# vliu15/3d-brain-tumor-segmentation

Hardware: AMD Instinct MI355X
Metric: training volumes/sec (2ch x 128^3) (higher is better)
Workload: dtype f32; 1 GPU; BASELINE configs[1]: 2ch x 128^3, batch 1 per GPU, fp32, full fwd+bwd with Dice+KL+L2 VAE loss + Dice metric + TF-form Adam; CLI-default model (base_filters=32, depth=4, groups=8, reduction=8; 42,174,773 params); parallelism=dp1, global_batch=1

## Files before the change

### 3d-brain-tumor-segmentation_amd/csrc/conv_c2.hip

```cpp
#include <stdlib.h>
#include "common.h"
#include "conv_plan.h"

struct C2Params {
  const float* x;
  const float* wp;
  const float* bias;
  float* y;
  const float* wp2;
  const float* bias2;
  float* y2;
  int N, D, H, W, ldx, Cout, ldy, ldy2, Npad;
  int ntz, nty, ntx;
  double* gnp;
  int gn_G, gn_zt;
};

template <bool F2>
__global__ __launch_bounds__(256, 2) void c2_kernel(const C2Params p) {
  __shared__ float lds[2 * 6 * 6 * 34 + 16];
  const int tid = threadIdx.x;
  const int lane = tid & 63;
  const int wave = __builtin_amdgcn_readfirstlane(tid >> 6);
  const int h = lane >> 5, l32 = lane & 31;
  int b = blockIdx.x;
  const int tx = b % p.ntx; b /= p.ntx;
  const int ty = b % p.nty; b /= p.nty;
  const int tz = b % p.ntz;
  const int n = b / p.ntz;
  const int oz0 = tz * 4, oy0 = ty * 4, ox0 = tx * 32;
  for (int e = tid; e < 6 * 6 * 34; e += 256) {
    const int vz = e / (6 * 34), r = e - vz * (6 * 34);
    const int vy = r / 34, vx = r - vy * 34;
    const int z = oz0 - 1 + vz, yy = oy0 - 1 + vy, xx = ox0 - 1 + vx;
    float v0 = 0.f, v1 = 0.f;
    if ((unsigned)z < (unsigned)p.D && (unsigned)yy < (unsigned)p.H && (unsigned)xx < (unsigned)p.W) {
      const float* s = p.x + ((((long)n * p.D + z) * p.H + yy) * p.W + xx) * (long)p.ldx;
      v0 = s[0]; v1 = s[1];
    }
    lds[e] = v0;
    lds[6 * 6 * 34 + e] = v1;
  }
  float wt[27];
#pragma unroll
  for (int t = 0; t < 27; ++t) wt[t] = p.wp[((long)t * 2 * p.Npad + l32) * 4 + h];
  float w2 = 0.f;
  if (F2) w2 = p.wp2[l32 * 4 + h];
  __syncthreads();
  f32x16 acc[4], acc2[F2 ? 4 : 1];
#pragma unroll
  for (int i = 0; i < 4; ++i)
#pragma unroll
    for (int r = 0; r < 16; ++r) { acc[i][r] = 0.f; if (F2) acc2[F2 ? i : 0][r] = 0.f; }
  const float* lb = lds + h * (6 * 6 * 34) + (wave * 6) * 34 + l32;
#pragma unroll
  for (int kz = 0; kz < 3; ++kz) {
    float f[6][3];
#pragma unroll
    for (int yr = 0; yr < 6; ++yr)
#pragma unroll
      for (int kx = 0; kx < 3; ++kx) f[yr][kx] = lb[(kz * 6 + yr) * 34 + kx];
#pragma unroll
    for (int ky = 0; ky < 3; ++ky)
#pragma unroll
      for (int kx = 0; kx < 3; ++kx)
#pragma unroll
        for (int oy = 0; oy < 4; ++oy)
          acc[oy] = __builtin_amdgcn_mfma_f32_32x32x2f32(wt[(kz * 3 + ky) * 3 + kx], f[oy + ky][kx], acc[oy], 0, 0, 0);
    if (F2 && kz == 1) {
#pragma unroll
      for (int oy = 0; oy < 4; ++oy) acc2[F2 ? oy : 0] = __builtin_amdgcn_mfma_f32_32x32x2f32(w2, f[oy + 1][1], acc2[F2 ? oy : 0], 0, 0, 0);
    }
  }
  const int oz = oz0 + wave, ox = ox0 + l32;
  float gn_s = 0.f, gn_q = 0.f;
  if (oz < p.D && ox < p.W) {
#pragma unroll
    for (int oy = 0; oy < 4; ++oy) {
      const int y = oy0 + oy;
      if (y >= p.H) continue;
      const long pix = (((long)n * p.D + oz) * p.H + y) * p.W + ox;
#pragma unroll
      for (int g = 0; g < 4; ++g) {
        const int co = 8 * g + 4 * h;
        if (co >= p.Cout) continue;
        f32x4 v = {acc[oy][4 * g], acc[oy][4 * g + 1], acc[oy][4 * g + 2], acc[oy][4 * g + 3]};
        if (p.bias) {
#pragma unroll
          for (int j = 0; j < 4; ++j) v[j] += p.bias[co + j];
        }
        if (p.gnp) {
#pragma unroll
          for (int j = 0; j < 4; ++j) { gn_s += v[j]; gn_q = fmaf(v[j], v[j], gn_q); }
        }
        *reinterpret_cast<f32x4*>(p.y + pix * p.ldy + co) = v;
        if (F2) {
          f32x4 v2 = {acc2[F2 ? oy : 0][4 * g], acc2[F2 ? oy : 0][4 * g + 1], acc2[F2 ? oy : 0][4 * g + 2], acc2[F2 ? oy : 0][4 * g + 3]};
          if (p.bias2) {
#pragma unroll
            for (int j = 0; j < 4; ++j) v2[j] += p.bias2[co + j];
          }
          *reinterpret_cast<f32x4*>(p.y2 + pix * p.ldy2 + co) = v2;
        }
      }
    }
  }
  if (p.gnp) {
    const double ds = wave_sum_f64((double)gn_s), dq = wave_sum_f64((double)gn_q);
    __syncthreads();
    double* sh = reinterpret_cast<double*>(lds);
    if (lane == 0) { sh[wave * 2] = ds; sh[wave * 2 + 1] = dq; }
    __syncthreads();
    if (tid == 0) {
      const int g = tz / p.gn_zt;
      const long B = (long)p.gn_zt * p.nty * p.ntx;
      const long b_ = ((long)(tz - g * p.gn_zt) * p.nty + ty) * p.ntx + tx;
      double* o = p.gnp + (((long)n * p.gn_G + g) * B + b_) * 2;
      o[0] = sh[0] + sh[2] + sh[4] + sh[6];
      o[1] = sh[1] + sh[3] + sh[5] + sh[7];
    }
  }
}

static inline long c2_tiles(const ConvCall& c, int& ntx, int& nty, int& ntz) {
  ntx = (c.Wi + 31) / 32; nty = (c.Hi + 3) / 4; ntz = (c.Di + 3) / 4;
  return (long)c.N * ntz * nty * ntx;
}
bool c2_accept(const ConvCall& c, ConvChoice& ch) {
  if (c.Cin != 2 || c.Cout > 32 || c.Cout % 4 != 0 || c.ldy % 4 != 0 || !c.y16) return false;
  if (c.flags & (IG_FLAG_ACCUM | IG_FLAG_SIGMOID)) return false;
  if (c.second == CONV_Y2 && (c.ld2 % 4 != 0 || !c.p2_16)) return false;
  int ntx, nty, ntz;
  const long tiles = c2_tiles(c, ntx, nty, ntz);
  if (tiles < conv_env_long("BTS_IGEMM_C2_MIN", 512) || tiles > 0x7fffffffL) return false;
  ch.sym = SYM_C2;
  ch.gn_B = (long)conv_gn_zt(c, 4) * nty * ntx;
  return true;
}
int bts_c2_launch_(const ConvCall& c, const ConvChoice& ch, const ConvPtrs& q, hipStream_t stream) {
  const bool f2 = c.second == CONV_Y2;
  C2Params p;
  p.x = q.x; p.wp = q.wp; p.bias = (c.flags & IG_FLAG_BIAS) ? q.bias : nullptr; p.y = q.y;
  p.wp2 = f2 ? q.wp2 : nullptr; p.bias2 = f2 ? q.bias2 : nullptr; p.y2 = f2 ? q.y2 : nullptr;
  p.N = c.N; p.D = c.Di; p.H = c.Hi; p.W = c.Wi; p.ldx = c.ldx; p.Cout = c.Cout; p.ldy = c.ldy; p.ldy2 = f2 ? c.ld2 : 0; p.Npad = conv_npad32(c.Cout);
  const long tiles = c2_tiles(c, p.ntx, p.nty, p.ntz);
  p.gnp = ch.gn_B ? q.gnp : nullptr; p.gn_G = ch.gn_B ? c.G : 0; p.gn_zt = ch.gn_B ? (c.Di / c.G) / 4 : 1;
  const bool prof = bts_prof_on();
  if (prof) bts_prof_begin(ch.sym, 2.0 * (27.0 + (f2 ? 1.0 : 0.0)) * c.Cin * (double)c.Cout * (double)c.N * c.Di * c.Hi * c.Wi, stream);
  (void)hipGetLastError();
  if (f2) hipLaunchKernelGGL(c2_kernel<true>, dim3((unsigned)tiles), dim3(256), 0, stream, p);
  else hipLaunchKernelGGL(c2_kernel<false>, dim3((unsigned)tiles), dim3(256), 0, stream, p);
  if (prof) bts_prof_end(stream);
  BTS_LAUNCH_CHECK();
  return BTS_OK;
}
```

### 3d-brain-tumor-segmentation_amd/csrc/conv_dsc.hip

```cpp
#include <stdlib.h>
#include "common.h"
#include "conv_plan.h"

struct DscParams {
  const float* x;
  const float* wp;
  const float* bias;
  float* y;
  int N, D, H, W, Cin, ldx, Cout, ldy, Npad, KG, ntx, nty, ntz, flags;
};
template <int CO>
__global__ __launch_bounds__(256, 4) void dsc_kernel(const DscParams p) {
  constexpr int S = 12, TX = 32, TY = 4, TZ = 2, IX = TX + 2, IY = TY + 2, IZ = TZ + 2;
  constexpr int tileVox = IZ * IY * IX, nslots = tileVox * 2, NSL = (nslots + 255) / 256;
  __shared__ __attribute__((aligned(16))) float lds[tileVox * S];
  const int tid = threadIdx.x;
  int b = blockIdx.x;
  const int tx = b % p.ntx; b /= p.ntx;
  const int ty = b % p.nty; b /= p.nty;
  const int tz = b % p.ntz;
  const int n = b / p.ntz;
  const int iz0 = tz * TZ - 1, iy0 = ty * TY - 1, ix0 = tx * TX - 1;
  const float* xbase = p.x + ((((long)n * p.D + iz0) * p.H + iy0) * p.W + ix0) * (long)p.ldx;
  int goff[NSL];
#pragma unroll
  for (int i = 0; i < NSL; ++i) {
    const int e = tid + i * 256;
    goff[i] = -1;
    if (e < nslots) {
      const int vox = e >> 1, q = e & 1;
      const int vz = vox / (IY * IX), r = vox - vz * (IY * IX), vy = r / IX, vx = r - vy * IX;
      if ((unsigned)(iz0 + vz) < (unsigned)p.D && (unsigned)(iy0 + vy) < (unsigned)p.H && (unsigned)(ix0 + vx) < (unsigned)p.W)
        goff[i] = ((vz * p.H + vy) * p.W + vx) * p.ldx + q * 4;
    }
  }
  const int mx = tid & (TX - 1), my = (tid >> 5) & (TY - 1), mz = tid >> 7;
  const float* lb = lds + ((mz * IY + my) * IX + mx) * S;
  float acc[CO];
#pragma unroll
  for (int c = 0; c < CO; ++c) acc[c] = 0.f;
  const int wstepKG = 2 * p.Npad * 4, wstepTap = p.KG * wstepKG;
  f32x4 pre[NSL];
  auto fetch = [&](int kg) {
#pragma unroll
    for (int i = 0; i < NSL; ++i) {
      f32x4 v = {0.f, 0.f, 0.f, 0.f};
      if (goff[i] >= 0) v = *reinterpret_cast<const f32x4*>(xbase + goff[i] + kg * 8);
      pre[i] = v;
    }
  };
  fetch(0);
  for (int kg = 0; kg < p.KG; ++kg) {
    __syncthreads();
#pragma unroll
    for (int i = 0; i < NSL; ++i) {
      const int e = tid + i * 256;
      if (e < nslots) *reinterpret_cast<f32x4*>(lds + (e >> 1) * S + (e & 1) * 4) = pre[i];
    }
    __syncthreads();
    if (kg + 1 < p.KG) fetch(kg + 1);
    const float* wk = p.wp + kg * wstepKG;
#pragma unroll
    for (int r = 0; r < 9; ++r) {
      float w[3][2][CO * 4];
#pragma unroll
      for (int dx = 0; dx < 3; ++dx)
#pragma unroll
        for (int hh = 0; hh < 2; ++hh)
#pragma unroll
          for (int q = 0; q < CO * 4; ++q) w[dx][hh][q] = wk[(r * 3 + dx) * wstepTap + hh * p.Npad * 4 + q];
      f32x4 xv[3][2];
#pragma unroll
      for (int dx = 0; dx < 3; ++dx) {
        const float* src = lb + (((r / 3) * IY + r % 3) * IX + dx) * S;
        xv[dx][0] = *reinterpret_cast<const f32x4*>(src);
        xv[dx][1] = *reinterpret_cast<const f32x4*>(src + 4);
      }
      __builtin_amdgcn_sched_barrier(0);
#pragma unroll
      for (int dx = 0; dx < 3; ++dx)
#pragma unroll
        for (int hh = 0; hh < 2; ++hh)
#pragma unroll
          for (int c = 0; c < CO; ++c)
#pragma unroll
            for (int j = 0; j < 4; ++j) acc[c] = fmaf(xv[dx][hh][j], w[dx][hh][c * 4 + j], acc[c]);
      __builtin_amdgcn_sched_barrier(0);
    }
  }
  const int oz = tz * TZ + mz, oy = ty * TY + my, ox = tx * TX + mx;
  if (oz >= p.D || oy >= p.H || ox >= p.W) return;
  float* yrow = p.y + ((((long)n * p.D + oz) * p.H + oy) * p.W + ox) * (long)p.ldy;
#pragma unroll
  for (int c = 0; c < CO; ++c) {
    if (c < p.Cout) {
      float v = acc[c];
      if (p.flags & IG_FLAG_BIAS) v += p.bias[c];
      if (p.flags & IG_FLAG_SIGMOID) v = sigmoidf_(v);
      if (p.flags & IG_FLAG_ACCUM) v += yrow[c];
      yrow[c] = v;
    }
  }
}

static inline long dsc_tiles(const ConvCall& c, int& ntx, int& nty, int& ntz) {
  ntx = (c.Wi + 31) / 32; nty = (c.Hi + 3) / 4; ntz = (c.Di + 1) / 2;
  return (long)c.N * ntz * nty * ntx;
}
bool dsc_accept(const ConvCall& c, ConvChoice& ch) {
  if (c.Cout > 4 || (c.Cin & 7) || (c.ldx & 3) || !c.x16) return false;
  int ntx, nty, ntz;
  const long tiles = dsc_tiles(c, ntx, nty, ntz);
  ch.sym = SYM_DSC;
  return tiles >= conv_env_long("BTS_IGEMM_DSC_MIN", 1024) && tiles <= 0x7fffffffL;
}
int bts_dsc_launch_(const ConvCall& c, const ConvChoice& ch, const ConvPtrs& q, hipStream_t stream) {
  DscParams p;
  p.x = q.x; p.wp = q.wp; p.bias = q.bias; p.y = q.y;
  p.N = c.N; p.D = c.Di; p.H = c.Hi; p.W = c.Wi; p.Cin = c.Cin; p.ldx = c.ldx; p.Cout = c.Cout; p.ldy = c.ldy;
  p.Npad = conv_npad32(c.Cout); p.KG = c.Cin / 8;
  p.flags = c.flags;
  const long tiles = dsc_tiles(c, p.ntx, p.nty, p.ntz);
  const bool prof = bts_prof_on();
  if (prof) bts_prof_begin(ch.sym, 2.0 * 27.0 * c.Cin * (double)c.Cout * (double)c.N * c.Di * c.Hi * c.Wi, stream);
  (void)hipGetLastError();
  if (c.Cout <= 2) hipLaunchKernelGGL(dsc_kernel<2>, dim3((unsigned)tiles), dim3(256), 0, stream, p);
  else hipLaunchKernelGGL(dsc_kernel<4>, dim3((unsigned)tiles), dim3(256), 0, stream, p);
  if (prof) bts_prof_end(stream);
  BTS_LAUNCH_CHECK();
  return BTS_OK;
}
```

Before: 29.42 volumes/s.

## Stream z-planes with rolling accumulators in small-Cout conv; transpose C2 fused MFMA

The small-Cout conv kernel now has each block march through a chunk of z-planes. It loads each input plane once into LDS and scatters its contribution into three rolling per-output accumulators, so the 3-deep halo in z is no longer reloaded for every 2-plane tile. It also stages up to 4 channel groups per LDS fill, uses packed 2-wide FMAs, reads weights through the constant address space, and sizes the grid to about 768 blocks. The Cin=2 conv with a fused 1x1 branch swaps its MFMA operands so each lane holds one output channel and writes scalar per-voxel outputs. The risks are fewer blocks and less parallelism, more register pressure, and strided scalar stores in the C2 path.

```diff
diff --git a/3d-brain-tumor-segmentation_amd/csrc/conv_c2.hip b/3d-brain-tumor-segmentation_amd/csrc/conv_c2.hip
--- a/3d-brain-tumor-segmentation_amd/csrc/conv_c2.hip
+++ b/3d-brain-tumor-segmentation_amd/csrc/conv_c2.hip
@@ -66,41 +66,58 @@
       for (int kx = 0; kx < 3; ++kx)
 #pragma unroll
         for (int oy = 0; oy < 4; ++oy)
-          acc[oy] = __builtin_amdgcn_mfma_f32_32x32x2f32(wt[(kz * 3 + ky) * 3 + kx], f[oy + ky][kx], acc[oy], 0, 0, 0);
+          acc[oy] = F2 ? __builtin_amdgcn_mfma_f32_32x32x2f32(f[oy + ky][kx], wt[(kz * 3 + ky) * 3 + kx], acc[oy], 0, 0, 0)
+                       : __builtin_amdgcn_mfma_f32_32x32x2f32(wt[(kz * 3 + ky) * 3 + kx], f[oy + ky][kx], acc[oy], 0, 0, 0);
     if (F2 && kz == 1) {
 #pragma unroll
-      for (int oy = 0; oy < 4; ++oy) acc2[F2 ? oy : 0] = __builtin_amdgcn_mfma_f32_32x32x2f32(w2, f[oy + 1][1], acc2[F2 ? oy : 0], 0, 0, 0);
+      for (int oy = 0; oy < 4; ++oy) acc2[F2 ? oy : 0] = __builtin_amdgcn_mfma_f32_32x32x2f32(f[oy + 1][1], w2, acc2[F2 ? oy : 0], 0, 0, 0);
     }
   }
-  const int oz = oz0 + wave, ox = ox0 + l32;
+  const int oz = oz0 + wave;
   float gn_s = 0.f, gn_q = 0.f;
-  if (oz < p.D && ox < p.W) {
+  if (F2) {
+    const int co = l32;
+    if (oz < p.D && co < p.Cout) {
+      const float bv = p.bias ? p.bias[co] : 0.f;
+      const float bv2 = p.bias2 ? p.bias2[co] : 0.f;
 #pragma unroll
-    for (int oy = 0; oy < 4; ++oy) {
-      const int y = oy0 + oy;
-      if (y >= p.H) continue;
-      const long pix = (((long)n * p.D + oz) * p.H + y) * p.W + ox;
+      for (int oy = 0; oy < 4; ++oy) {
+        const int y = oy0 + oy;
+        if (y >= p.H) continue;
+        const long row = (((long)n * p.D + oz) * p.H + y) * p.W;
 #pragma unroll
-      for (int g = 0; g < 4; ++g) {
-        const int co = 8 * g + 4 * h;
-        if (co >= p.Cout) continue;
-        f32x4 v = {acc[oy][4 * g], acc[oy][4 * g + 1], acc[oy][4 * g + 2], acc[oy][4 * g + 3]};
-        if (p.bias) {
+        for (int r = 0; r < 16; ++r) {
+          const int ox = ox0 + 8 * (r >> 2) + 4 * h + (r & 3);
+          if (ox >= p.W) continue;
+          const float v = acc[oy][r] + bv;
+          if (p.gnp) { gn_s += v; gn_q = fmaf(v, v, gn_q); }
+          p.y[(row + ox) * p.ldy + co] = v;
+          p.y2[(row + ox) * p.ldy2 + co] = acc2[F2 ? oy : 0][r] + bv2;
+        }
+      }
+    }
+  } else {
+    const int ox = ox0 + l32;
+    if (oz < p.D && ox < p.W) {
 #pragma unroll
-          for (int j = 0; j < 4; ++j) v[j] += p.bias[co + j];
-        }
-        if (p.gnp) {
+      for (int oy = 0; oy < 4; ++oy) {
+        const int y = oy0 + oy;
+        if (y >= p.H) continue;
+        const long pix = (((long)n * p.D + oz) * p.H + y) * p.W + ox;
 #pragma unroll
-          for (int j = 0; j < 4; ++j) { gn_s += v[j]; gn_q = fmaf(v[j], v[j], gn_q); }
-        }
-        *reinterpret_cast<f32x4*>(p.y + pix * p.ldy + co) = v;
-        if (F2) {
-          f32x4 v2 = {acc2[F2 ? oy : 0][4 * g], acc2[F2 ? oy : 0][4 * g + 1], acc2[F2 ? oy : 0][4 * g + 2], acc2[F2 ? oy : 0][4 * g + 3]};
-          if (p.bias2) {
+        for (int g = 0; g < 4; ++g) {
+          const int co = 8 * g + 4 * h;
+          if (co >= p.Cout) continue;
+          f32x4 v = {acc[oy][4 * g], acc[oy][4 * g + 1], acc[oy][4 * g + 2], acc[oy][4 * g + 3]};
+          if (p.bias) {
 #pragma unroll
-            for (int j = 0; j < 4; ++j) v2[j] += p.bias2[co + j];
+            for (int j = 0; j < 4; ++j) v[j] += p.bias[co + j];
           }
-          *reinterpret_cast<f32x4*>(p.y2 + pix * p.ldy2 + co) = v2;
+          if (p.gnp) {
+#pragma unroll
+            for (int j = 0; j < 4; ++j) { gn_s += v[j]; gn_q = fmaf(v[j], v[j], gn_q); }
+          }
+          *reinterpret_cast<f32x4*>(p.y + pix * p.ldy + co) = v;
         }
       }
     }
diff --git a/3d-brain-tumor-segmentation_amd/csrc/conv_dsc.hip b/3d-brain-tumor-segmentation_amd/csrc/conv_dsc.hip
--- a/3d-brain-tumor-segmentation_amd/csrc/conv_dsc.hip
+++ b/3d-brain-tumor-segmentation_amd/csrc/conv_dsc.hip
@@ -7,110 +7,154 @@
   const float* wp;
   const float* bias;
   float* y;
-  int N, D, H, W, Cin, ldx, Cout, ldy, Npad, KG, ntx, nty, ntz, flags;
+  int N, D, H, W, Cin, ldx, Cout, ldy, KG, KC, lq, ntx, nty, nzc, ZC, flags;
 };
+typedef float f32x2 __attribute__((ext_vector_type(2)));
+typedef const __attribute__((address_space(4))) float* dsc_wptr;
+constexpr int DSC_TX = 32, DSC_TY = 8;
+constexpr int DSC_NPAD = 32;
 template <int CO>
-__global__ __launch_bounds__(256, 4) void dsc_kernel(const DscParams p) {
-  constexpr int S = 12, TX = 32, TY = 4, TZ = 2, IX = TX + 2, IY = TY + 2, IZ = TZ + 2;
-  constexpr int tileVox = IZ * IY * IX, nslots = tileVox * 2, NSL = (nslots + 255) / 256;
+__global__ __launch_bounds__(256, 3) void dsc_kernel(const DscParams p) {
+  constexpr int S = 36, TX = DSC_TX, TY = DSC_TY, IX = TX + 2, IY = TY + 2;
+  constexpr int tileVox = IY * IX, NSL = (tileVox * 8 + 255) / 256;
   __shared__ __attribute__((aligned(16))) float lds[tileVox * S];
   const int tid = threadIdx.x;
   int b = blockIdx.x;
   const int tx = b % p.ntx; b /= p.ntx;
   const int ty = b % p.nty; b /= p.nty;
-  const int tz = b % p.ntz;
-  const int n = b / p.ntz;
-  const int iz0 = tz * TZ - 1, iy0 = ty * TY - 1, ix0 = tx * TX - 1;
-  const float* xbase = p.x + ((((long)n * p.D + iz0) * p.H + iy0) * p.W + ix0) * (long)p.ldx;
+  const int zc = b % p.nzc;
+  const int n = b / p.nzc;
+  const int z0 = zc * p.ZC, z1 = min(z0 + p.ZC, p.D);
+  const int zlo = max(z0 - 1, 0), zhi = min(z1, p.D - 1);
+  const int iy0 = ty * TY - 1, ix0 = tx * TX - 1;
+  const float* xbase = p.x + (((long)n * p.D * p.H + iy0) * p.W + ix0) * (long)p.ldx;
+  const long xplane = (long)p.H * p.W * p.ldx;
+  const int nslots = tileVox << p.lq;
   int goff[NSL];
 #pragma unroll
   for (int i = 0; i < NSL; ++i) {
     const int e = tid + i * 256;
     goff[i] = -1;
     if (e < nslots) {
-      const int vox = e >> 1, q = e & 1;
-      const int vz = vox / (IY * IX), r = vox - vz * (IY * IX), vy = r / IX, vx = r - vy * IX;
-      if ((unsigned)(iz0 + vz) < (unsigned)p.D && (unsigned)(iy0 + vy) < (unsigned)p.H && (unsigned)(ix0 + vx) < (unsigned)p.W)
-        goff[i] = ((vz * p.H + vy) * p.W + vx) * p.ldx + q * 4;
+      const int vox = e >> p.lq, q = e & ((1 << p.lq) - 1);
+      const int vy = vox / IX, vx = vox - vy * IX;
+      if ((unsigned)(iy0 + vy) < (unsigned)p.H && (unsigned)(ix0 + vx) < (unsigned)p.W) goff[i] = (vy * p.W + vx) * p.ldx + q * 4;
     }
   }
-  const int mx = tid & (TX - 1), my = (tid >> 5) & (TY - 1), mz = tid >> 7;
-  const float* lb = lds + ((mz * IY + my) * IX + mx) * S;
-  float acc[CO];
+  const int mx = tid & (TX - 1), my = tid >> 5;
+  const float* lb0 = lds + (my * IX + mx) * S;
+  const int oy = ty * TY + my, ox = tx * TX + mx;
+  const bool live = oy < p.H && ox < p.W;
+  float* ycol = p.y + (((long)n * p.D * p.H + oy) * p.W + ox) * (long)p.ldy;
+  const long yplane = (long)p.H * p.W * p.ldy;
+  f32x2 acc[3][CO];
 #pragma unroll
-  for (int c = 0; c < CO; ++c) acc[c] = 0.f;
-  const int wstepKG = 2 * p.Npad * 4, wstepTap = p.KG * wstepKG;
+  for (int a = 0; a < 3; ++a)
+#pragma unroll
+    for (int c = 0; c < CO; ++c) acc[a][c] = f32x2{0.f, 0.f};
+  constexpr int wstepKG = 2 * DSC_NPAD * 4;
+  const int wstepTap = p.KG * wstepKG;
   f32x4 pre[NSL];
-  auto fetch = [&](int kg) {
+  auto fetch = [&](int zi, int kg) {
+    const float* xs = xbase + zi * xplane + kg * 8;
 #pragma unroll
     for (int i = 0; i < NSL; ++i) {
       f32x4 v = {0.f, 0.f, 0.f, 0.f};
-      if (goff[i] >= 0) v = *reinterpret_cast<const f32x4*>(xbase + goff[i] + kg * 8);
+      if (goff[i] >= 0) v = *reinterpret_cast<const f32x4*>(xs + goff[i]);
       pre[i] = v;
     }
   };
-  fetch(0);
-  for (int kg = 0; kg < p.KG; ++kg) {
-    __syncthreads();
+  auto retire = [&](int zo) {
+    if (!live) return;
+    float* yrow = ycol + zo * yplane;
+#pragma unroll
+    for (int c = 0; c < CO; ++c) {
+      if (c < p.Cout) {
+        float v = acc[0][c].x + acc[0][c].y;
+        if (p.flags & IG_FLAG_BIAS) v += p.bias[c];
+        if (p.flags & IG_FLAG_SIGMOID) v = sigmoidf_(v);
+        if (p.flags & IG_FLAG_ACCUM) v += yrow[c];
+        yrow[c] = v;
+      }
+    }
+  };
+  fetch(zlo, 0);
+  int zi = zlo, kg0 = 0;
+  for (bool first = true;; first = false) {
+    if (!first) __syncthreads();
 #pragma unroll
     for (int i = 0; i < NSL; ++i) {
       const int e = tid + i * 256;
-      if (e < nslots) *reinterpret_cast<f32x4*>(lds + (e >> 1) * S + (e & 1) * 4) = pre[i];
+      if (e < nslots) *reinterpret_cast<f32x4*>(lds + (e >> p.lq) * S + (e & ((1 << p.lq) - 1)) * 4) = pre[i];
     }
     __syncthreads();
-    if (kg + 1 < p.KG) fetch(kg + 1);
-    const float* wk = p.wp + kg * wstepKG;
+    const bool lastkg = kg0 + p.KC == p.KG;
+    if (!lastkg || zi < zhi) fetch(lastkg ? zi + 1 : zi, lastkg ? 0 : kg0 + p.KC);
+    for (int kl = 0; kl < p.KC; ++kl) {
+      const float* lb = lb0 + kl * 8;
+      const dsc_wptr wk = (dsc_wptr)(p.wp + (kg0 + kl) * wstepKG);
 #pragma unroll
-    for (int r = 0; r < 9; ++r) {
-      float w[3][2][CO * 4];
+      for (int dy = 0; dy < 3; ++dy) {
+        f32x4 xv[3][2];
 #pragma unroll
-      for (int dx = 0; dx < 3; ++dx)
+        for (int dx = 0; dx < 3; ++dx) {
+          const float* src = lb + (dy * IX + dx) * S;
+          xv[dx][0] = *reinterpret_cast<const f32x4*>(src);
+          xv[dx][1] = *reinterpret_cast<const f32x4*>(src + 4);
+        }
 #pragma unroll
-        for (int hh = 0; hh < 2; ++hh)
+        for (int kz = 0; kz < 3; ++kz) {
+          const int zo = zi + 1 - kz;
+          if (zo < z0 || zo >= z1) continue;
+          float w[3][2][CO * 4];
 #pragma unroll
-          for (int q = 0; q < CO * 4; ++q) w[dx][hh][q] = wk[(r * 3 + dx) * wstepTap + hh * p.Npad * 4 + q];
-      f32x4 xv[3][2];
+          for (int dx = 0; dx < 3; ++dx)
 #pragma unroll
-      for (int dx = 0; dx < 3; ++dx) {
-        const float* src = lb + (((r / 3) * IY + r % 3) * IX + dx) * S;
-        xv[dx][0] = *reinterpret_cast<const f32x4*>(src);
-        xv[dx][1] = *reinterpret_cast<const f32x4*>(src + 4);
+            for (int hh = 0; hh < 2; ++hh)
+#pragma unroll
+              for (int q = 0; q < CO * 4; ++q) w[dx][hh][q] = wk[((kz * 3 + dy) * 3 + dx) * wstepTap + hh * DSC_NPAD * 4 + q];
+          __builtin_amdgcn_sched_barrier(0);
+#pragma unroll
+          for (int dx = 0; dx < 3; ++dx)
+#pragma unroll
+            for (int hh = 0; hh < 2; ++hh)
+#pragma unroll
+              for (int c = 0; c < CO; ++c)
+#pragma unroll
+                for (int j = 0; j < 4; j += 2)
+                  acc[2 - kz][c] = __builtin_elementwise_fma(f32x2{xv[dx][hh][j], xv[dx][hh][j + 1]},
+                                                             f32x2{w[dx][hh][c * 4 + j], w[dx][hh][c * 4 + j + 1]}, acc[2 - kz][c]);
+          __builtin_amdgcn_sched_barrier(0);
+        }
       }
-      __builtin_amdgcn_sched_barrier(0);
+    }
+    if (lastkg) {
+      if (zi - 1 >= z0) retire(zi - 1);
 #pragma unroll
-      for (int dx = 0; dx < 3; ++dx)
-#pragma unroll
-        for (int hh = 0; hh < 2; ++hh)
-#pragma unroll
-          for (int c = 0; c < CO; ++c)
-#pragma unroll
-            for (int j = 0; j < 4; ++j) acc[c] = fmaf(xv[dx][hh][j], w[dx][hh][c * 4 + j], acc[c]);
-      __builtin_amdgcn_sched_barrier(0);
+      for (int c = 0; c < CO; ++c) { acc[0][c] = acc[1][c]; acc[1][c] = acc[2][c]; acc[2][c] = f32x2{0.f, 0.f}; }
+      if (zi == zhi) break;
+      ++zi; kg0 = 0;
+    } else {
+      kg0 += p.KC;
     }
   }
-  const int oz = tz * TZ + mz, oy = ty * TY + my, ox = tx * TX + mx;
-  if (oz >= p.D || oy >= p.H || ox >= p.W) return;
-  float* yrow = p.y + ((((long)n * p.D + oz) * p.H + oy) * p.W + ox) * (long)p.ldy;
-#pragma unroll
-  for (int c = 0; c < CO; ++c) {
-    if (c < p.Cout) {
-      float v = acc[c];
-      if (p.flags & IG_FLAG_BIAS) v += p.bias[c];
-      if (p.flags & IG_FLAG_SIGMOID) v = sigmoidf_(v);
-      if (p.flags & IG_FLAG_ACCUM) v += yrow[c];
-      yrow[c] = v;
-    }
-  }
+  if (zhi < z1) retire(zhi);
 }
 
-static inline long dsc_tiles(const ConvCall& c, int& ntx, int& nty, int& ntz) {
-  ntx = (c.Wi + 31) / 32; nty = (c.Hi + 3) / 4; ntz = (c.Di + 1) / 2;
-  return (long)c.N * ntz * nty * ntx;
+static inline long dsc_tiles(const ConvCall& c) {
+  return (long)c.N * ((c.Di + 1) / 2) * ((c.Hi + 3) / 4) * ((c.Wi + 31) / 32);
+}
+static inline long dsc_grid(const ConvCall& c, DscParams& p) {
+  p.ntx = (c.Wi + DSC_TX - 1) / DSC_TX; p.nty = (c.Hi + DSC_TY - 1) / DSC_TY;
+  const long cols = (long)c.N * p.nty * p.ntx;
+  const long runs = std::max(1L, (768 + cols - 1) / cols);
+  p.ZC = (int)std::min<long>(c.Di, std::max(4L, (c.Di + runs - 1) / runs));
+  p.nzc = (c.Di + p.ZC - 1) / p.ZC;
+  return cols * p.nzc;
 }
 bool dsc_accept(const ConvCall& c, ConvChoice& ch) {
   if (c.Cout > 4 || (c.Cin & 7) || (c.ldx & 3) || !c.x16) return false;
-  int ntx, nty, ntz;
-  const long tiles = dsc_tiles(c, ntx, nty, ntz);
+  const long tiles = dsc_tiles(c);
   ch.sym = SYM_DSC;
   return tiles >= conv_env_long("BTS_IGEMM_DSC_MIN", 1024) && tiles <= 0x7fffffffL;
 }
@@ -118,9 +162,11 @@
   DscParams p;
   p.x = q.x; p.wp = q.wp; p.bias = q.bias; p.y = q.y;
   p.N = c.N; p.D = c.Di; p.H = c.Hi; p.W = c.Wi; p.Cin = c.Cin; p.ldx = c.ldx; p.Cout = c.Cout; p.ldy = c.ldy;
-  p.Npad = conv_npad32(c.Cout); p.KG = c.Cin / 8;
+  p.KG = c.Cin / 8;
+  p.KC = (p.KG % 4 == 0) ? 4 : (p.KG % 2 == 0) ? 2 : 1;
+  p.lq = p.KC == 4 ? 3 : p.KC == 2 ? 2 : 1;
   p.flags = c.flags;
-  const long tiles = dsc_tiles(c, p.ntx, p.nty, p.ntz);
+  const long tiles = dsc_grid(c, p);
   const bool prof = bts_prof_on();
   if (prof) bts_prof_begin(ch.sym, 2.0 * 27.0 * c.Cin * (double)c.Cout * (double)c.N * c.Di * c.Hi * c.Wi, stream);
   (void)hipGetLastError();
```

Result: no change. 29.61 volumes/s, median of 3 (+0.7%).
